# dask-contrib/dask-sql

Hardware: NVIDIA H100
Metric: rows/s on Q3-shaped filter->join->groupby (higher is better)
Workload: dtype f64

## Files before the change

### dask-sql_b200/_lib.py

```python
import ctypes as C
import os

HERE = os.path.dirname(os.path.abspath(__file__))
LIB_PATH = os.environ.get("B200SQL_LIB") or os.path.join(HERE, "libb200sql.so")

I64, F64, U8 = 0, 1, 2
U32 = 3
COL_SENTINEL = 1
MAX_COLS, MAX_TERMS, MAX_AGGS, MAX_KEYS, MAX_GATHER, MAX_PROG = 16, 8, 8, 4, 8, 64
TILE = 4096
EQ, NE, LT, LE, GT, GE, IS_NULL, IS_NOT_NULL, IS_TRUE = range(9)
AGG_SUM, AGG_SUMF, AGG_MIN, AGG_MAX, AGG_COUNT, AGG_AND, AGG_OR, AGG_XOR = range(8)
JOIN_INNER, JOIN_LEFT, JOIN_SEMI, JOIN_ANTI = range(4)
EMPTY_KEY = -(1 << 63)

OP_LOAD, OP_CONST_I, OP_CONST_F, OP_CONST_NULL, OP_I2F, OP_F2I = 0, 1, 2, 3, 4, 5
OP_ADD_I, OP_SUB_I, OP_MUL_I, OP_DIV_I, OP_NEG_I, OP_ABS_I, OP_MOD_I = 10, 11, 12, 13, 14, 15, 16
OP_ADD_F, OP_SUB_F, OP_MUL_F, OP_DIV_F, OP_NEG_F, OP_ABS_F, OP_SQRT_F = 20, 21, 22, 23, 24, 25, 26
OP_EQ_I, OP_EQ_F = 30, 40
OP_AND, OP_OR, OP_NOT, OP_ISNULL_I, OP_ISNULL_F, OP_CASE, OP_FILLNA, OP_ORD2F = 50, 51, 52, 53, 54, 55, 56, 57


class Col(C.Structure):
    _fields_ = [("data", C.c_void_p), ("valid", C.c_void_p), ("dtype", C.c_int32), ("flags", C.c_int32)]
# ... 11 lines not shown

class Agg(C.Structure):
    _fields_ = [("col", C.c_int32), ("op", C.c_int32)]


class AggState(C.Structure):
    _fields_ = [("acc", C.c_void_p * MAX_AGGS), ("cnt", C.c_void_p * MAX_AGGS), ("rows", C.c_void_p),
                ("present", C.c_void_p), ("out_slot", C.c_void_p)]


class Instr(C.Structure):
    _fields_ = [("op", C.c_int32), ("a", C.c_int32), ("imm_i", C.c_int64), ("imm_f", C.c_double)]


class Prog(C.Structure):
    _fields_ = [("code", Instr * MAX_PROG), ("n", C.c_int32), ("out_dtype", C.c_int32)]


class JoinTable(C.Structure):
    _fields_ = [("keys", Col * MAX_KEYS), ("nkeys", C.c_int32), ("dense", C.c_int32), ("head", C.c_void_p),
                ("next", C.c_void_p), ("cap", C.c_int64), ("lookup", C.c_void_p), ("kmin", C.c_int64),
                ("range", C.c_int64)]


JA_P, JA_B, JA_MUL, JA_ADD, JA_SUB, JA_RSUB, JA_ROWS = range(7)
JA_MAX_BUILD = 4


class JoinAgg(C.Structure):
    _fields_ = [("pcol", C.c_int32), ("bcol", C.c_int32), ("combine", C.c_int32), ("op", C.c_int32)]


class StarLookup(C.Structure):
    _fields_ = [("dense", C.c_int32), ("pad_", C.c_int32), ("lookup", C.c_void_p), ("kmin", C.c_int64),
                ("range", C.c_int64), ("table_keys", C.c_void_p), ("table_slots", C.c_void_p),
                ("cap", C.c_int64), ("dir", C.c_void_p)]


MAX_PEERS, PEER_MAX_ARRAYS = 16, 2 * MAX_AGGS + 1
PEER_SUM_F64, PEER_SUM_I64, PEER_MIN_I64, PEER_MAX_I64, PEER_AND_I64, PEER_OR_I64, PEER_XOR_I64 = range(7)
PEER_PRESENT_ROWS, PEER_PRESENT_INDICATOR, PEER_PRESENT_BITMAP = 1, 2, 3


class PeerMerge(C.Structure):
    _fields_ = [("world", C.c_int32), ("rank", C.c_int32), ("narrays", C.c_int32), ("presence_kind", C.c_int32),
                ("presence_array", C.c_int32), ("ops", C.c_int32 * PEER_MAX_ARRAYS),
                ("array_off", C.c_int64 * PEER_MAX_ARRAYS), ("bitmap_off", C.c_int64), ("signal_off", C.c_int64),
                ("peer_base", C.c_void_p * MAX_PEERS), ("out", C.c_void_p * PEER_MAX_ARRAYS),
                ("out_present", C.c_void_p), ("lo", C.c_int64), ("count", C.c_int64), ("local_ready", C.c_void_p),
                ("epoch", C.c_uint64)]


assert C.sizeof(Col) == 24 and C.sizeof(Term) == 32 and C.sizeof(Scan) == 656
assert C.sizeof(AggState) == 152 and C.sizeof(Instr) == 24 and C.sizeof(Prog) == 1544
assert C.sizeof(JoinTable) == 152 and C.sizeof(StarLookup) == 64 and C.sizeof(PeerMerge) == 544


def agg_identity(op):
    return {AGG_MIN: (1 << 63) - 1, AGG_MAX: -(1 << 63), AGG_AND: -1}.get(op, 0)


class B200SqlError(RuntimeError):
    pass


def _load():
    if not os.path.exists(LIB_PATH):
# ... 51 lines not shown
    "b2_join_count": [C.POINTER(Scan), C.POINTER(C.c_int32), C.POINTER(JoinTable), C.c_int32, _P, _P],
    "b2_join_write": [C.POINTER(Scan), C.POINTER(C.c_int32), C.POINTER(JoinTable), C.c_int32, _P, _P, _P,
                      _P, _P],
    "b2_join_write_gather": [C.POINTER(Scan), C.POINTER(C.c_int32), C.POINTER(JoinTable), C.c_int32, _P, _P, _P,
                             _P, C.c_int32, C.POINTER(C.c_int32), C.POINTER(_P), C.POINTER(_P), C.c_int32,
                             C.POINTER(Col), C.POINTER(_P), C.POINTER(_P), _P],
    "b2_join_key_layout": [C.POINTER(Col), C.c_int64, C.c_int64, C.c_int64, C.POINTER(Col), C.c_int32, C.c_int64,
                           _P, _P, _P, _P],
    "b2_join_write_gather_keyed": [C.POINTER(Scan), C.POINTER(C.c_int32), C.POINTER(JoinTable), C.c_int32, _P, _P,
                                   _P, _P, C.c_int32, C.POINTER(C.c_int32), C.POINTER(_P), C.POINTER(_P),
                                   C.c_int32, C.POINTER(Col), C.POINTER(C.c_int64), C.POINTER(_P), C.POINTER(_P),
                                   _P],
    "b2_join_onepass": [C.POINTER(Scan), C.POINTER(C.c_int32), C.POINTER(JoinTable), C.c_int32, C.c_int32, _P, C.c_int32,
                        C.POINTER(C.c_int32), C.POINTER(_P), C.POINTER(_P), C.c_int32, C.POINTER(Col),
                        C.POINTER(C.c_int64), C.POINTER(_P), C.POINTER(_P), _P],
    "b2_join_agg": [C.POINTER(Scan), C.c_int32, C.POINTER(JoinTable), C.c_int32, C.POINTER(Col), C.POINTER(C.c_int64),
                    C.POINTER(JoinAgg), C.c_int32, _P, _P, C.c_int32, _P, _P],
    "b2_range_partition_hist": [C.POINTER(Scan), C.c_int32, C.c_int64, C.c_int64, C.c_int32, C.c_int32, _P, _P],
    "b2_range_partition_scan": [C.c_int32, _P, _P],
    "b2_range_partition_scatter": [C.POINTER(Scan), C.c_int32, C.c_int64, C.c_int64, C.c_int32, C.c_int32, C.c_int32,
                                   C.POINTER(C.c_int32), _P, C.POINTER(_P), _P, _P],
    "b2_range_partition": [C.POINTER(Scan), C.c_int32, C.c_int64, C.c_int64, C.c_int32, C.c_int32, C.c_int32,
                           C.POINTER(C.c_int32), _P, C.POINTER(_P), _P, _P],
    "b2_iota": [_P, C.c_int64, _P],
    "b2_bitwise_combine": [_P, _P, C.c_int64, C.c_int32, _P],
    "b2_peer_merge": [C.POINTER(PeerMerge), _P],
    "b2_sort_by": [C.POINTER(Col), C.c_int64, C.c_int32, C.c_int32, _P, _P, _P],
    "b2_dense_slots": [C.POINTER(Col), C.c_int64, C.c_int64, C.c_int32, _P, _P],
    "b2_star_build_dense": [C.POINTER(Col), _P, C.c_int64, _P, C.c_int64, C.c_int64, _P, _P, _P],
    "b2_star_build_mark": [C.POINTER(Scan), C.c_int32, C.c_int64, C.c_int64, _P, _P, _P],
    "b2_star_build_rank": [_P, C.c_int64, _P],
    "b2_star_build_fill": [C.POINTER(Scan), C.c_int32, C.c_int32, C.c_int64, C.c_int64, C.c_int64, C.c_int32, _P,
                           _P, _P],
    "b2_star_build_hash": [C.POINTER(Col), _P, C.c_int64, _P, _P, _P, C.c_int64, _P, _P],
    "b2_star_agg": [C.POINTER(Scan), C.c_int32, C.POINTER(StarLookup), C.POINTER(Agg), C.c_int32,
                    C.POINTER(AggState), _P],
}

EXPORTS = sorted(list(_SIGS) + ["b2_last_error", "b2_num_tiles", "b2_stats_ws_bytes", "b2_scan_agg_ws_bytes",
                                "b2_sort_ws_bytes", "b2_join_onepass_ws_bytes", "b2_range_partition_ws_bytes",
                                "b2_f64_to_ordered", "b2_ordered_to_f64"])


call_times = {} if os.environ.get("B200SQL_CALL_TIMES") == "1" else None


def _wrap(name):
    fn = getattr(_lib, name)
    fn.restype = C.c_int32
    fn.argtypes = _SIGS[name]

    if call_times is not None:
        import time

        def call(*args):
            t0 = time.perf_counter()
            rc = fn(*args)
            rec = call_times.setdefault(name, [0, 0.0])
            rec[0] += 1
            rec[1] += time.perf_counter() - t0
            if rc != 0:
                raise B200SqlError(f"{name} failed ({rc}): {_lib.b2_last_error().decode()}")
            return rc

        call.__name__ = name
        return call
# ... 24 lines not shown
groupby_dense_ordered = _wrap("b2_groupby_dense_ordered")
groupby_dense_grouped = _wrap("b2_groupby_dense_grouped")
groupby_dense_hot = _wrap("b2_groupby_dense_hot")
hot_slots = _wrap("b2_hot_slots")
groupby_hash1 = _wrap("b2_groupby_hash1")
groupby_hashk = _wrap("b2_groupby_hashk")
join_build = _wrap("b2_join_build")
join_build_dense = _wrap("b2_join_build_dense")
join_count = _wrap("b2_join_count")
join_write = _wrap("b2_join_write")
join_write_gather = _wrap("b2_join_write_gather")
join_write_gather_keyed = _wrap("b2_join_write_gather_keyed")
join_key_layout = _wrap("b2_join_key_layout")
join_onepass = _wrap("b2_join_onepass")
join_onepass_ws_bytes = _lib.b2_join_onepass_ws_bytes
join_agg = _wrap("b2_join_agg")
range_partition = _wrap("b2_range_partition")
range_partition_hist = _wrap("b2_range_partition_hist")
range_partition_scan = _wrap("b2_range_partition_scan")
range_partition_scatter = _wrap("b2_range_partition_scatter")
range_partition_ws_bytes = _lib.b2_range_partition_ws_bytes
iota = _wrap("b2_iota")
bitwise_combine = _wrap("b2_bitwise_combine")
peer_merge = _wrap("b2_peer_merge")
sort_by = _wrap("b2_sort_by")
_lib.b2_sort_ws_bytes.restype = C.c_int64
_lib.b2_sort_ws_bytes.argtypes = [C.c_int64]
sort_ws_bytes = _lib.b2_sort_ws_bytes
dense_slots = _wrap("b2_dense_slots")
star_build_dense = _wrap("b2_star_build_dense")
star_build_mark = _wrap("b2_star_build_mark")
star_build_rank = _wrap("b2_star_build_rank")
star_build_fill = _wrap("b2_star_build_fill")
star_build_hash = _wrap("b2_star_build_hash")
star_agg = _wrap("b2_star_agg")
num_tiles = _lib.b2_num_tiles
stats_ws_bytes = _lib.b2_stats_ws_bytes
scan_agg_ws_bytes = _lib.b2_scan_agg_ws_bytes
f64_to_ordered = _lib.b2_f64_to_ordered
ordered_to_f64 = _lib.b2_ordered_to_f64


def has_symbol(name):
    try:
        getattr(_lib, name)
        return True
    except AttributeError:
        return False
```

### dask-sql_b200/csrc/groupby.cuh

```cuda
#pragma once
#include "common.cuh"
#include "pipeline.cuh"
#include "warpagg.cuh"

#define B2_GB_R 8
#define B2_GB_ROWS_PER_BLOCK (B2_BLOCK * B2_GB_R)
#define B2_MAX_PROBE 1024

template <int R, class LD>
__device__ __forceinline__ void b2_dense_slots_of(const b2_scan_t& s, const LD& ld, int key_col, int64_t kmin,
                                                  int64_t nslots, int64_t (&slot)[R]) {
  const b2_col_t& kc = s.cols[key_col];
  bool full;
  const uint32_t bits = b2_eval_terms<R>(s, ld, full);
  int64_t key[R];
  ld.template load<R>(key_col, bits, full, key);
  uint32_t kvalid = bits;
  if (kc.valid) kvalid = b2_valid_bits<R>(kc.valid, ld.row0, bits);
#pragma unroll
  for (int j = 0; j < R; ++j) {
    slot[j] = -1;
    if ((bits >> j) & 1) {
      if (!((kvalid >> j) & 1)) slot[j] = nslots - 1;
      else {
// ... 191 lines not shown
                        const __grid_constant__ b2_keys_arg keys, int64_t* __restrict__ tk,
                        uint8_t* __restrict__ tnull, int32_t* __restrict__ tstate, int64_t cap,
                        const __grid_constant__ b2_aggs_arg aggs, const __grid_constant__ b2_aggstate_t st,
                        int32_t* __restrict__ flags) {
  auto body = [&](const auto& ld) { b2_hashk_body(s, ld, keys, tk, tnull, tstate, cap, aggs, st, flags); };
  if (PIPE) b2_tile_pipeline(s, pp, body);
  else b2_tile_direct<B2_GB_R>(s, body);
}

__global__ void __launch_bounds__(B2_BLOCK)
b2_dense_slots_kernel(const __grid_constant__ b2_col_t key, int64_t n, int64_t kmin, int32_t null_slot,
                      int32_t* __restrict__ out) {
  for (int64_t i = (int64_t)blockIdx.x * B2_BLOCK + threadIdx.x; i < n; i += (int64_t)gridDim.x * B2_BLOCK) {
    const int64_t raw = b2_load_raw(key, i);
    out[i] = b2_is_null(key, i, raw) ? null_slot : (int32_t)(raw - kmin);
  }
}

__global__ void __launch_bounds__(B2_BLOCK)
b2_star_build_dense_kernel(const __grid_constant__ b2_col_t pk, const int32_t* __restrict__ sel, int64_t n_sel,
                           const int32_t* __restrict__ slot_of_row, int64_t kmin, int64_t range,
                           int32_t* __restrict__ lookup, int32_t* __restrict__ flags) {
  for (int64_t i = (int64_t)blockIdx.x * B2_BLOCK + threadIdx.x; i < n_sel; i += (int64_t)gridDim.x * B2_BLOCK) {
    const int64_t r = sel ? sel[i] : i;
    const int64_t raw = b2_load_raw(pk, r);
    if (b2_is_null(pk, r, raw)) continue;
    const uint64_t d = (uint64_t)raw - (uint64_t)kmin;
    if (d >= (uint64_t)range) continue;
    const int32_t old = atomicExch(lookup + d, slot_of_row[i]);
    if (old != -1) flags[0] = 1;
  }
}

template <bool FILL>
__global__ void __launch_bounds__(B2_BLOCK)
b2_star_build_scan_kernel(const __grid_constant__ b2_scan_t s, int pk_col, int grp_col, int64_t pk_min,
                          int64_t pk_range, int64_t grp_min, int32_t null_slot, uint64_t* __restrict__ dir,
                          int32_t* __restrict__ slots, int32_t* __restrict__ flags) {
  const int tile_off = (threadIdx.x >> 5) * (32 * B2_GB_R) + (threadIdx.x & 31);
  const b2_col_t& pc = s.cols[pk_col];
  const b2_col_t& gc = s.cols[grp_col];
  for (int64_t base = (int64_t)blockIdx.x * B2_GB_ROWS_PER_BLOCK; base < s.n;
       base += (int64_t)gridDim.x * B2_GB_ROWS_PER_BLOCK) {
    const b2_gld ld{&s, base + tile_off};
    bool full;
    const uint32_t bits = b2_eval_terms<B2_GB_R>(s, ld, full);
    int64_t pk[B2_GB_R];
    ld.template load<B2_GB_R>(pk_col, bits, full, pk);
    uint32_t live = bits;
    if (pc.valid) live &= b2_valid_bits<B2_GB_R>(pc.valid, ld.row0, bits);
#pragma unroll
    for (int j = 0; j < B2_GB_R; ++j) {
      const uint64_t d = (uint64_t)pk[j] - (uint64_t)pk_min;
      if (!(((live >> j) & 1) && d < (uint64_t)pk_range)) live &= ~(1u << j);
    }
    if (!FILL) {
#pragma unroll
      for (int j = 0; j < B2_GB_R; ++j) {
        if (!((live >> j) & 1)) continue;
        const uint64_t d = (uint64_t)pk[j] - (uint64_t)pk_min;
        const uint32_t b = 1u << (d & 31);
        if (atomicOr(reinterpret_cast<uint32_t*>(dir + (d >> 5)), b) & b) flags[0] = 1;
      }
    } else {
      int64_t grp[B2_GB_R];
      ld.template load<B2_GB_R>(grp_col, live, false, grp);
      uint32_t gnull = 0;
      if (gc.valid) gnull = live & ~b2_valid_bits<B2_GB_R>(gc.valid, ld.row0, live);
#pragma unroll
      for (int j = 0; j < B2_GB_R; ++j) {
        if (!((live >> j) & 1)) continue;
        const uint64_t d = (uint64_t)pk[j] - (uint64_t)pk_min;
        const uint64_t w = dir[d >> 5];
        const uint32_t pos = (uint32_t)(w >> 32) + __popc((uint32_t)w & ((1u << (d & 31)) - 1));
        slots[pos] = (gnull >> j) & 1 ? null_slot : (int32_t)(grp[j] - grp_min);
      }
    }
  }
}

struct b2_scan_io_dir {
  uint64_t* dir;
  __device__ int64_t get(int64_t i) const { return __popc((uint32_t)dir[i]); }
  __device__ void put(int64_t i, int64_t v) const { dir[i] = (uint64_t)(uint32_t)dir[i] | ((uint64_t)v << 32); }
};

__global__ void __launch_bounds__(B2_SCAN_THREADS) b2_star_build_rank_kernel(uint64_t* __restrict__ dir, int64_t nwords) {
  b2_block_exclusive_scan(b2_scan_io_dir{dir}, nwords);
}

__global__ void __launch_bounds__(B2_BLOCK)
b2_star_build_hash_kernel(const __grid_constant__ b2_col_t pk, const int32_t* __restrict__ sel, int64_t n_sel,
                          const int32_t* __restrict__ slot_of_row, int64_t* __restrict__ tk,
                          int32_t* __restrict__ ts, int64_t cap, int32_t* __restrict__ flags) {
  for (int64_t i = (int64_t)blockIdx.x * B2_BLOCK + threadIdx.x; i < n_sel; i += (int64_t)gridDim.x * B2_BLOCK) {
    const int64_t r = sel ? sel[i] : i;
    const int64_t key = b2_load_raw(pk, r);
    if (b2_is_null(pk, r, key)) continue;
    if (key == B2_EMPTY_KEY) { flags[1] = 1; continue; }
    uint64_t h = b2_mix64((uint64_t)key) & (uint64_t)(cap - 1);
    bool done = false;
    for (int probe = 0; probe < B2_MAX_PROBE && !done; ++probe) {
      const unsigned long long old = atomicCAS(reinterpret_cast<unsigned long long*>(tk + h),
                                               (unsigned long long)B2_EMPTY_KEY, (unsigned long long)key);
      if (old == (unsigned long long)B2_EMPTY_KEY) { ts[h] = slot_of_row[i]; done = true; }
      else if (old == (unsigned long long)key) { flags[0] = 1; done = true; }
      else h = (h + 1) & (uint64_t)(cap - 1);
    }
// ... 2 lines not shown
}

__device__ __forceinline__ int32_t b2_star_lookup(const b2_starlookup_t& lk, int64_t key) {
  if (lk.dense) {
    const uint64_t d = (uint64_t)key - (uint64_t)lk.kmin;
    return d < (uint64_t)lk.range ? b2_ld_keep_i32(lk.lookup + d) : -1;
  }
  uint64_t h = b2_mix64((uint64_t)key) & (uint64_t)(lk.cap - 1);
  for (int probe = 0; probe < B2_MAX_PROBE; ++probe) {
    const int64_t cur = __ldg(reinterpret_cast<const long long*>(lk.table_keys) + h);
    if (cur == key) return b2_ld_keep_i32(lk.table_slots + h);
    if (cur == B2_EMPTY_KEY) return -1;
    h = (h + 1) & (uint64_t)(lk.cap - 1);
  }
  return -1;
}

#define B2_STAR_R 16
template <int R, class LD>
__device__ __forceinline__ void b2_star_body(const b2_scan_t& s, const LD& ld, int fk_col, const b2_starlookup_t& lk,
                                             const b2_aggs_arg& aggs, const b2_aggstate_t& st) {
  const b2_col_t& kc = s.cols[fk_col];
  bool full0;
  const uint32_t inb = b2_bounds_bits<R>(ld.row0, s.n, full0);
  int64_t key[R];
  ld.template load<R>(fk_col, inb, full0, key);
  bool full;
  const uint32_t bits = b2_eval_terms<R>(s, ld, full);
  uint32_t live = bits;
  if (kc.valid) live &= b2_valid_bits<R>(kc.valid, ld.row0, bits);
  const bool prefetch = aggs.n > 0 && aggs.a[0].col >= 0;
  int64_t pre[R];
  int32_t found[R];
  if (lk.dense == 2) {
    const uint64_t range = (uint64_t)lk.range;
    uint64_t w[R];
#pragma unroll
    for (int j = 0; j < R; ++j) {
      const uint64_t d = (uint64_t)key[j] - (uint64_t)lk.kmin;
      w[j] = (((live >> j) & 1) && d < range) ? (uint64_t)b2_ld_keep_i64(reinterpret_cast<const int64_t*>(lk.dir) + (d >> 5)) : 0;
    }
    if (prefetch) ld.template load<R>(aggs.a[0].col, live, false, pre);
#pragma unroll
    for (int j = 0; j < R; ++j) {
      const uint32_t b = (uint32_t)((uint64_t)key[j] - (uint64_t)lk.kmin) & 31;
      const uint32_t bits = (uint32_t)w[j];
      found[j] = (bits >> b) & 1 ? b2_ld_keep_i32(lk.lookup + (uint32_t)(w[j] >> 32) + __popc(bits & ((1u << b) - 1))) : -1;
    }
  } else if (lk.dense) {
    const uint64_t range = (uint64_t)lk.range;
#pragma unroll
    for (int j = 0; j < R; ++j) {
      const uint64_t d = (uint64_t)key[j] - (uint64_t)lk.kmin;
      found[j] = (((live >> j) & 1) && d < range) ? b2_ld_keep_i32(lk.lookup + d) : -1;
    }
  } else {
#pragma unroll
    for (int j = 0; j < R; ++j) {
      found[j] = -1;
      if (((live >> j) & 1) && key[j] != B2_EMPTY_KEY) found[j] = b2_star_lookup(lk, key[j]);
    }
  }
  if (lk.dense != 2 && prefetch) ld.template load<R>(aggs.a[0].col, live, false, pre);
  int64_t slot[R];
#pragma unroll
  for (int j = 0; j < R; ++j) slot[j] = found[j];
  b2_apply_aggs<R>(s, ld, aggs.a, aggs.n, st, slot, pre);
}

template <bool PIPE>
__global__ void __launch_bounds__(PIPE ? B2_PIPE_THREADS : B2_BLOCK)
b2_star_agg_kernel(const __grid_constant__ b2_scan_t s, const __grid_constant__ b2_pipe_t pp, int fk_col,
                   const __grid_constant__ b2_starlookup_t lk, const __grid_constant__ b2_aggs_arg aggs,
                   const __grid_constant__ b2_aggstate_t st) {
  if (PIPE) b2_tile_pipeline(s, pp, [&](const auto& ld) { b2_star_body<B2_PIPE_R>(s, ld, fk_col, lk, aggs, st); });
  else b2_tile_direct<B2_STAR_R>(s, [&](const auto& ld) { b2_star_body<B2_STAR_R>(s, ld, fk_col, lk, aggs, st); });
}

extern "C" {

static int32_t b2_check_state(const b2_aggs_arg& aa, const b2_aggstate_t* st) {
  B2_REQUIRE(st, "null aggstate");
  for (int a = 0; a < aa.n; ++a) {
    if (aa.a[a].col < 0) { B2_REQUIRE(st->rows, "COUNT(*) needs aggstate.rows"); continue; }
    if (aa.a[a].op == B2_AGG_COUNT) B2_REQUIRE(st->cnt[a], "COUNT needs a cnt array");
    else B2_REQUIRE(st->acc[a], "aggregate needs an acc array");
  }
  return B2_OK;
}
static inline bool b2_pow2(int64_t x) { return x > 0 && (x & (x - 1)) == 0; }

static int32_t b2_groupby_dense_impl(const b2_scan_t* scan, int32_t key_col, int64_t kmin, int64_t nslots,
                                     const b2_agg_t* aggs, int32_t naggs, const b2_aggstate_t* st,
                                     unsigned long long* ticket, void* stream) {
  int32_t rc = b2_check_scan(scan);
  if (rc) return rc;
  b2_aggs_arg aa;
// ... 156 lines not shown
    int64_t nblk = (scan->n + B2_GB_ROWS_PER_BLOCK - 1) / B2_GB_ROWS_PER_BLOCK;
    int grid = b2_wave_grid(b2_groupby_hashk_kernel<false>, B2_BLOCK, nblk);
    b2_groupby_hashk_kernel<false><<<grid, B2_BLOCK, 0, (cudaStream_t)stream>>>(*scan, pp, ka, table_keys, table_nulls,
                                                                        table_state, cap, aa, *st, d_flags);
  }
  B2_CHECK_LAUNCH("b2_groupby_hashk_kernel");
  return B2_OK;
}

int32_t b2_dense_slots(const b2_col_t* key, int64_t n, int64_t kmin, int32_t null_slot, int32_t* out_slot,
                       void* stream) {
  B2_REQUIRE(key && out_slot, "null argument");
  if (n <= 0) return B2_OK;
  int grid = b2_wave_grid(b2_dense_slots_kernel, B2_BLOCK, (n + B2_BLOCK - 1) / B2_BLOCK);
  b2_dense_slots_kernel<<<grid, B2_BLOCK, 0, (cudaStream_t)stream>>>(*key, n, kmin, null_slot, out_slot);
  B2_CHECK_LAUNCH("b2_dense_slots_kernel");
  return B2_OK;
}

int32_t b2_star_build_dense(const b2_col_t* pk, const int32_t* sel, int64_t n_sel, const int32_t* slot_of_row,
                            int64_t kmin, int64_t range, int32_t* lookup, int32_t* d_flags, void* stream) {
  B2_REQUIRE(pk && slot_of_row && lookup && d_flags, "null argument");
  B2_REQUIRE(pk->dtype == B2_I64, "dense lookup needs an int64 key");
  if (n_sel <= 0) return B2_OK;
  int grid = b2_wave_grid(b2_star_build_dense_kernel, B2_BLOCK, (n_sel + B2_BLOCK - 1) / B2_BLOCK);
  b2_star_build_dense_kernel<<<grid, B2_BLOCK, 0, (cudaStream_t)stream>>>(*pk, sel, n_sel, slot_of_row, kmin,
                                                                           range, lookup, d_flags);
  B2_CHECK_LAUNCH("b2_star_build_dense_kernel");
  return B2_OK;
}

static int32_t b2_star_build_pass(bool fill, const b2_scan_t* scan, int32_t pk_col, int32_t grp_col,
                                  int64_t pk_min, int64_t pk_range, int64_t grp_min, int32_t null_slot,
                                  uint64_t* dir, int32_t* slots, int32_t* d_flags, void* stream) {
  int32_t rc = b2_check_scan(scan);
  if (rc) return rc;
  B2_REQUIRE(pk_col >= 0 && pk_col < scan->ncols && grp_col >= 0 && grp_col < scan->ncols, "column out of range");
  B2_REQUIRE(scan->cols[pk_col].dtype == B2_I64 && scan->cols[grp_col].dtype == B2_I64, "dense keys must be int64");
  B2_REQUIRE(pk_range > 0 && pk_range < ((int64_t)1 << 31), "bad range");
  if (scan->n == 0) return B2_OK;
  int64_t nblk = (scan->n + B2_GB_ROWS_PER_BLOCK - 1) / B2_GB_ROWS_PER_BLOCK;
  if (fill) {
    int grid = b2_wave_grid(b2_star_build_scan_kernel<true>, B2_BLOCK, nblk);
    b2_star_build_scan_kernel<true><<<grid, B2_BLOCK, 0, (cudaStream_t)stream>>>(*scan, pk_col, grp_col, pk_min, pk_range,
                                                                                  grp_min, null_slot, dir, slots, d_flags);
  } else {
    int grid = b2_wave_grid(b2_star_build_scan_kernel<false>, B2_BLOCK, nblk);
    b2_star_build_scan_kernel<false><<<grid, B2_BLOCK, 0, (cudaStream_t)stream>>>(*scan, pk_col, grp_col, pk_min, pk_range,
                                                                                   grp_min, null_slot, dir, slots, d_flags);
  }
  B2_CHECK_LAUNCH("b2_star_build_scan_kernel");
  return B2_OK;
}

int32_t b2_star_build_mark(const b2_scan_t* scan, int32_t pk_col, int64_t pk_min, int64_t pk_range, uint64_t* dir,
                           int32_t* d_flags, void* stream) {
  B2_REQUIRE(dir && d_flags, "null argument");
  return b2_star_build_pass(false, scan, pk_col, pk_col, pk_min, pk_range, 0, 0, dir, nullptr, d_flags, stream);
}

int32_t b2_star_build_rank(uint64_t* dir, int64_t pk_range, void* stream) {
  B2_REQUIRE(dir, "null argument");
  B2_REQUIRE(pk_range > 0 && pk_range < ((int64_t)1 << 31), "bad range");
  b2_star_build_rank_kernel<<<1, B2_SCAN_THREADS, 0, (cudaStream_t)stream>>>(dir, (pk_range + 31) / 32);
  B2_CHECK_LAUNCH("b2_star_build_rank_kernel");
  return B2_OK;
}

int32_t b2_star_build_fill(const b2_scan_t* scan, int32_t pk_col, int32_t grp_col, int64_t pk_min,
                           int64_t pk_range, int64_t grp_min, int32_t null_slot, const uint64_t* dir,
                           int32_t* slots, void* stream) {
  B2_REQUIRE(dir && slots, "null argument");
  return b2_star_build_pass(true, scan, pk_col, grp_col, pk_min, pk_range, grp_min, null_slot,
                            const_cast<uint64_t*>(dir), slots, nullptr, stream);
}

int32_t b2_star_build_hash(const b2_col_t* pk, const int32_t* sel, int64_t n_sel, const int32_t* slot_of_row,
                           int64_t* table_keys, int32_t* table_slots, int64_t cap, int32_t* d_flags,
                           void* stream) {
  B2_REQUIRE(pk && slot_of_row && table_keys && table_slots && d_flags, "null argument");
  B2_REQUIRE(pk->dtype == B2_I64, "star lookup needs an int64 key");
  B2_REQUIRE(b2_pow2(cap), "cap must be a power of two");
  if (n_sel <= 0) return B2_OK;
  int grid = b2_wave_grid(b2_star_build_hash_kernel, B2_BLOCK, (n_sel + B2_BLOCK - 1) / B2_BLOCK);
  b2_star_build_hash_kernel<<<grid, B2_BLOCK, 0, (cudaStream_t)stream>>>(*pk, sel, n_sel, slot_of_row, table_keys,
                                                                          table_slots, cap, d_flags);
  B2_CHECK_LAUNCH("b2_star_build_hash_kernel");
  return B2_OK;
}

int32_t b2_star_agg(const b2_scan_t* scan, int32_t fk_col, const b2_starlookup_t* lk, const b2_agg_t* aggs,
                    int32_t naggs, const b2_aggstate_t* st, void* stream) {
  int32_t rc = b2_check_scan(scan);
  if (rc) return rc;
  b2_aggs_arg aa;
  if ((rc = b2_check_aggs(scan, aggs, naggs, &aa))) return rc;
  if ((rc = b2_check_state(aa, st))) return rc;
  B2_REQUIRE(lk, "null lookup");
  B2_REQUIRE(fk_col >= 0 && fk_col < scan->ncols, "fk column out of range");
  B2_REQUIRE(scan->cols[fk_col].dtype == B2_I64, "fk must be int64");
  B2_REQUIRE(lk->dense >= 0 && lk->dense <= 2, "bad lookup kind");
  if (lk->dense == 2) B2_REQUIRE(lk->dir && lk->lookup && lk->range > 0 && lk->range < ((int64_t)1 << 31), "bad bitmap lookup");
  else if (lk->dense) B2_REQUIRE(lk->lookup && lk->range > 0, "bad dense lookup");
  else B2_REQUIRE(lk->table_keys && lk->table_slots && b2_pow2(lk->cap), "bad hash lookup");
  if (scan->n == 0) return B2_OK;
  b2_pipe_t pp;
  b2_make_pipe(*scan, &pp);
  if (pp.enabled) {
    int grid = b2_pipe_grid(b2_star_agg_kernel<true>, pp, scan->n);
    b2_star_agg_kernel<true><<<grid, B2_PIPE_THREADS, pp.smem_bytes, (cudaStream_t)stream>>>(*scan, pp, fk_col, *lk, aa, *st);
  } else {
    int64_t nblk = (scan->n + (int64_t)B2_BLOCK * B2_STAR_R - 1) / ((int64_t)B2_BLOCK * B2_STAR_R);
    int grid = b2_wave_grid(b2_star_agg_kernel<false>, B2_BLOCK, nblk);
    b2_star_agg_kernel<false><<<grid, B2_BLOCK, 0, (cudaStream_t)stream>>>(*scan, pp, fk_col, *lk, aa, *st);
  }
  B2_CHECK_LAUNCH("b2_star_agg_kernel");
  return B2_OK;
}

}
```

### dask-sql_b200/executor.py

```python
import ctypes as C
import os
from typing import Dict, List, Optional, Sequence, Set

import numpy as np
import torch

from . import _lib as L
from . import device as D
from . import expr as E
from . import parallel as P
from .device import DeviceColumn, TermSpec, I64, F64, U8
from .expr import Expr, ColRef, Lit, Call
from .frame import LazyFrame, Source, TableSource, JoinSource, AggSource, SortSource, LimitSource
from .table import DeviceTable, HostColumn

DENSE_MAX_SLOTS = 1 << 27
_TORCH_DT = {I64: torch.int64, F64: torch.float64, U8: torch.uint8}
_LOGICAL = {I64: "int64", F64: "float64", U8: "bool"}

stats = {"launches": 0, "star_fused": 0, "dense_groupby": 0, "hash_groupby": 0, "dense_join": 0,
         "chain_join": 0, "keyed_join": 0, "partitioned_groupby": 0, "h2d_bytes": 0, "d2h_bytes": 0}


kernel_events = None
# ... 1468 lines not shown
        self.gname = src.group_cols[0]
        self.gexpr0 = gexpr0
        self.glog = dim.col_type(gexpr0.name)[1] if isinstance(gexpr0, ColRef) else "int64"
        self.plan = AggPlan([(E.substitute(e, fact.exprs) if e is not None else None, o, f) for e, o, f in aggs],
                            _nullable_fn(fact, sharded))
        if any(not isinstance(ka.expr, ColRef) for ka in self.plan.kaggs):
            raise _NotPreparable()
        self.keep = []
        self.dim_launch = []
        if owner:
            needed = {pk_e.name, ge.name}
            for p in dpred:
                p.refs(needed)
            for part in self._resident_parts(dim.source.table, needed):
                ctx = ScanCtx(part, dpred)
                pk_slot, g_slot = ctx.slot(pk_e), ctx.slot(ge)
                self._only_table_columns(ctx)
                self.dim_launch.append((ctx.scan(), pk_slot, g_slot))
                self.keep.append(ctx)
        needed = set(fk_e.refs())
        for ka in self.plan.kaggs:
            ka.expr.refs(needed)
        for p in fpred:
            p.refs(needed)
        self.fact_launch = []
        for part in self._resident_parts(fact.source.table, needed):
            ctx = ScanCtx(part, fpred)
            fk_slot = ctx.slot(fk_e)
            specs = [(ctx.slot(ka.expr), ka.op) for ka in self.plan.kaggs]
            self._only_table_columns(ctx)
            self.fact_launch.append((ctx.scan(), fk_slot, D.make_aggs(specs), len(specs), part.n))
            self.keep.append(ctx)
        self.dn = dn
        _, self.flags_off, words = _star_bitmap_words(self.prange, dn)
        self.lookup = torch.empty(words, dtype=torch.int32, device=dev)
        self.lk = _star_bitmap_lookup(self.lookup, self.pmin, self.prange, dn)
        self.tabs = [GroupState(dev, self.nslots, self.plan, need_present=True,
                                alloc=_padded_slots(self.nslots, sharded))]
        self.refill = [self._refill_list(self.tabs[0].table)]
        self.dirty = [False]
        self.peer = None
        self.epoch = 0
        self.free = [None, None]
        self.merge_bufs = {}
        self.runs = 0

    @staticmethod
    def _refill_list(t: D.GroupTable):
        out = []
        for acc in t.acc:
            if acc is not None:
                out.append((acc, float(acc[0].item()) if acc.dtype == torch.float64 else int(acc[0].item())))
        for cnt in t.cnt:
            if cnt is not None:
                out.append((cnt, 0))
        if t.rows is not None:
            out.append((t.rows, 0))
        if t.present is not None:
            out.append((t.present, 0))
        return out

    def install_peer_merge(self, state):
        self.tabs, self.refill, self.dirty, self.peer, self.arena, self.local_ready = state
        stats["peer_merge_plans"] = stats.get("peer_merge_plans", 0) + 1

    def build_peer_merge(self):
        rank, size = P.world()
        dev = self.dev
        alloc = _padded_slots(self.nslots, True)
# ... 59 lines not shown

    @staticmethod
    def _resident_parts(table, needed):
        parts = []
        for p in table.partitions:
            n = next(iter(p.values())).n if p else 0
            if n == 0:
                continue
            cols = {}
            for name in needed:
                c = p[name]
                if not isinstance(c, DeviceColumn):
                    raise _NotPreparable()
                cols[name] = c
            parts.append(Part(cols, n))
        return parts

    @staticmethod
    def _only_table_columns(ctx: "ScanCtx"):
        if any(not k.startswith("col:") for k in ctx.index):
            raise _NotPreparable()

    def run(self, src) -> Part:
        i = self.runs & 1
        self.runs += 1
        buf = self.lookup
        main = D.cur_stream()
        sp = D.stream_ptr()
        if self.free[i] is not None:
            self.free[i].synchronize()
        if self.owner:
            with _Phase("build"):
                _star_bitmap_build(buf, self.dim_launch, self.pmin, self.prange, self.gmin, self.nslots - 1,
                                   self.dn, sp)
        if self.bcast:
            with _Phase("bcast"):
                P.broadcast_(buf, 0)
        ti = i if self.peer is not None else 0
        t = self.tabs[ti].table
        with _Phase("scan"):
            if self.dirty[ti]:
                for tensor, value in self.refill[ti]:
                    tensor.fill_(value)
            self.dirty[ti] = True
            for scan, fk_slot, aggs_arr, naggs, n in self.fact_launch:
                stats["launches"] += 1
                ev = _kernel_event_begin("b2_star_agg_kernel", n)
                L.star_agg(C.byref(scan), fk_slot, C.byref(self.lk), aggs_arr, naggs, C.byref(t.state), sp)
                _kernel_event_end(ev)
        if self.peer is not None:
            m, view = self.peer[ti]
            self.epoch += 1
            m.epoch = self.epoch
            with _Phase("peer_merge"):
                stats["launches"] += 1
                ev = _kernel_event_begin("b2_peer_merge_kernel", m.count)
                L.peer_merge(C.byref(m), sp)
                _kernel_event_end(ev)
        else:
            view = _merge_dense(t, self.plan, self.sharded, self.dev, keep=self.merge_bufs)
        stats["star_fused"] += 1

        def general():
            stats["star_fused"] -= 1
            return run_aggregate(src, allow_fast=False)

        out = _finalize_dense(view, self.gmin, self.gname, self.gexpr0, self.glog, self.plan, self.dev,
                              key_nullable=self.gnull, check=buf[self.flags_off:], fallback=general)
        done = torch.cuda.Event()
        done.record(main)
        self.free[i] = done
        return out


class _NotPreparable(Exception):
    pass


def _star_bitmap_words(prange, dn):
    slots = 2 * ((prange + 31) // 32)
    flags = slots + min(dn, prange)
    return slots, flags, flags + 4


def _star_bitmap_lookup(buf, pmin, prange, dn):
    lk = L.StarLookup()
    lk.dense, lk.dir, lk.kmin, lk.range = 2, buf.data_ptr(), pmin, prange
    lk.lookup = buf.data_ptr() + 4 * _star_bitmap_words(prange, dn)[0]
    return lk


def _star_bitmap_build(buf, launches, pmin, prange, gmin, null_slot, dn, sp):
    slots_off, flags_off, _ = _star_bitmap_words(prange, dn)
    base = buf.data_ptr()
    dirp, slots, flags = C.c_void_p(base), C.c_void_p(base + 4 * slots_off), C.c_void_p(base + 4 * flags_off)
    L.memset(dirp, 0, 4 * slots_off, sp)
    L.memset(flags, 0, 16, sp)
    for scan, pk_slot, _ in launches:
        stats["launches"] += 1
        L.star_build_mark(C.byref(scan), pk_slot, pmin, prange, dirp, flags, sp)
    stats["launches"] += 1
    L.star_build_rank(dirp, prange, sp)
    for scan, pk_slot, g_slot in launches:
        stats["launches"] += 1
        L.star_build_fill(C.byref(scan), pk_slot, g_slot, pmin, prange, gmin, null_slot, dirp, slots, sp)


def _star_dense_fast(src, fact, dim, fk_e, pk_e, gexprs, aggs, fact_pred, dim_pred, sharded, dev) -> Optional[Part]:
    if len(gexprs) != 1 or not isinstance(dim.source, TableSource) or not isinstance(pk_e, ColRef):
        return None
    ge = E.substitute(gexprs[0], dim.exprs)
    if not isinstance(ge, ColRef) or ge.dtype != I64 or pk_e.dtype != I64:
        return None
    rank, world = P.world()
    dist = frame_distribution(dim)
    if world > 1 and dist == "sharded":
        return None
    table = dim.source.table
    owner = world == 1 or dist != "root" or rank == 0
    meta = None
    if owner:
        pst, gst = table.column_stats(pk_e.name), table.column_stats(ge.name)
        gnull = table.column_nullable(ge.name)
        meta = (pst.vmin, pst.vmax, gst.vmin, gst.vmax, table.nrows, gnull)
    if world > 1 and dist == "root":
        cache = table.__dict__.setdefault("_root_meta", {})
        ck = (pk_e.name, ge.name)
        if ck not in cache:
            cache[ck] = P.broadcast_object(meta, 0)
        meta = cache[ck]
    pmin, pmax, gmin, gmax, dn, gnull = meta
    if pmin is None or gmin is None or dn == 0:
        return None
    prange, grng = pmax - pmin + 1, gmax - gmin + 1
    if not (prange <= max(4 * dn, 1 << 16) and prange < (1 << 31)):
        return None
    if not (grng + 1 <= DENSE_MAX_SLOTS and grng <= 8 * dn + 1024):
        return None
    dpred, never = simplify_pred(dim.pred + [E.substitute(p, dim.exprs) for p in dim_pred])
    fpred, fnever = simplify_pred(fact.pred + [E.substitute(p, fact.exprs) for p in fact_pred])
    if never or fnever:
        return None
    nslots = grng + 1
    if os.environ.get("B200SQL_NO_PREPARED") != "1":
        prep = PreparedStar.get(src, fact, dim, fk_e, pk_e, ge, gexprs[0], aggs, fpred, dpred,
                                (pmin, prange, gmin, grng, gnull, dn), owner, world > 1 and dist == "root", sharded, dev)
        if prep is not None:
            return prep.run(src)
    _, flags_off, words = _star_bitmap_words(prange, dn)
    buf = torch.empty(words, dtype=torch.int32, device=dev)
    flags = buf[flags_off:]
    with _Phase("build"):
        if owner:
            needed: Set[str] = {pk_e.name, ge.name}
            for p in dpred:
                p.refs(needed)
            launches, keep = [], []
            for part in materialize(dim.source, needed):
                if part.n == 0:
                    continue
                ctx = ScanCtx(part, dpred)
                pk_slot, g_slot = ctx.slot(pk_e), ctx.slot(ge)
                launches.append((ctx.scan(), pk_slot, g_slot))
                keep.append(ctx)
            _star_bitmap_build(buf, launches, pmin, prange, gmin, nslots - 1, dn, D.stream_ptr())
    if world > 1 and dist == "root":
        with _Phase("bcast"):
            P.broadcast_(buf, 0)
    plan = AggPlan([(E.substitute(e, fact.exprs) if e is not None else None, o, f) for e, o, f in aggs],
                   _nullable_fn(fact, sharded))
    gs = GroupState(dev, nslots, plan, need_present=True, alloc=_padded_slots(nslots, sharded))
    lk = _star_bitmap_lookup(buf, pmin, prange, dn)
    needed = set(fk_e.refs())
    for ka in plan.kaggs:
        ka.expr.refs(needed)
    for p in fpred:
        p.refs(needed)
    with _Phase("scan"):
        for part in materialize(fact.source, needed, pred=fpred):
            if part.n == 0:
                continue
            ctx = ScanCtx(part, fpred)
            fk_slot = ctx.slot(fk_e)
            gs.bind(ctx)
            stats["launches"] += 1
            ev = _kernel_event_begin("b2_star_agg_kernel", part.n)
            L.star_agg(C.byref(ctx.scan()), fk_slot, C.byref(lk), gs.table.aggs, len(gs.table.specs),
                       C.byref(gs.table.state), D.stream_ptr())
            _kernel_event_end(ev)
    view = _merge_dense(gs.table, plan, sharded, dev)
    glog = dim.col_type(gexprs[0].name)[1] if isinstance(gexprs[0], ColRef) else "int64"
    stats["star_fused"] += 1

    def general():
        stats["star_fused"] -= 1
        return run_aggregate(src, allow_fast=False)

    return _finalize_dense(view, gmin, src.group_cols[0], gexprs[0], glog, plan, dev, key_nullable=gnull,
                           check=flags, fallback=general)


def try_star(src: AggSource, child: LazyFrame, gexprs, aggs, pred, sharded, allow_fast=True) -> Optional[Part]:
    js: JoinSource = child.source
    if js.how != "inner" or len(js.left_on) != 1 or any(fn.lower() in MOMENT_FUNCS for _, _, fn in aggs):
        return None
# ... 467 lines not shown
```

### include/b200sql.h

```cpp
#ifndef B200SQL_H
#define B200SQL_H
#include <stdint.h>
#ifdef __cplusplus
extern "C" {
#endif

#define B2_OK            0
#define B2_ERR_CUDA     -1
#define B2_ERR_ARG      -2

#define B2_I64 0
#define B2_F64 1
#define B2_U8  2
#define B2_U32 3

#define B2_MAX_COLS   16
#define B2_MAX_TERMS   8
#define B2_MAX_AGGS    8
#define B2_MAX_KEYS    4
#define B2_MAX_GATHER  8
#define B2_MAX_PROG   64
#define B2_TILE     4096

#define B2_EQ 0
// ... 256 lines not shown
                    int64_t* d_out_acc, int64_t* d_out_cnt, int32_t accumulate, void* ws, void* stream);

int32_t b2_groupby_dense_ordered(const b2_scan_t* scan, int32_t key_col, int64_t kmin, int64_t nslots,
                                 const b2_agg_t* aggs, int32_t naggs, const b2_aggstate_t* st, uint64_t* d_ticket,
                                 void* stream);
int64_t b2_range_partition_ws_bytes(int32_t nbuckets);
int32_t b2_range_partition_hist(const b2_scan_t* scan, int32_t key_col, int64_t kmin, int64_t nslots, int32_t shift,
                                int32_t nbuckets, void* d_ws, void* stream);
int32_t b2_range_partition_scan(int32_t nbuckets, void* d_ws, void* stream);
int32_t b2_range_partition_scatter(const b2_scan_t* scan, int32_t key_col, int64_t kmin, int64_t nslots, int32_t shift,
                                   int32_t nbuckets, int32_t ncarry, const int32_t* carry_cols, int64_t* out_key,
                                   void* const* out_cols, void* d_ws, void* stream);
int32_t b2_range_partition(const b2_scan_t* scan, int32_t key_col, int64_t kmin, int64_t nslots, int32_t shift,
                           int32_t nbuckets, int32_t ncarry, const int32_t* carry_cols, int64_t* out_key,
                           void* const* out_cols, void* d_ws, void* stream);

int64_t b2_sort_ws_bytes(int64_t n);
int32_t b2_iota(int32_t* out, int64_t n, void* stream);
int32_t b2_sort_by(const b2_col_t* col, int64_t n, int32_t descending, int32_t nulls_first, int32_t* idx,
                   void* ws, void* stream);

int32_t b2_dense_slots(const b2_col_t* key, int64_t n, int64_t kmin, int32_t null_slot,
                       int32_t* out_slot, void* stream);

int32_t b2_star_build_dense(const b2_col_t* pk, const int32_t* sel, int64_t n_sel,
                            const int32_t* slot_of_row, int64_t kmin, int64_t range,
                            int32_t* lookup, int32_t* d_flags, void* stream);
int32_t b2_star_build_mark(const b2_scan_t* scan, int32_t pk_col, int64_t pk_min, int64_t pk_range,
                           uint64_t* dir, int32_t* d_flags, void* stream);
int32_t b2_star_build_rank(uint64_t* dir, int64_t pk_range, void* stream);
int32_t b2_star_build_fill(const b2_scan_t* scan, int32_t pk_col, int32_t grp_col, int64_t pk_min,
                           int64_t pk_range, int64_t grp_min, int32_t null_slot, const uint64_t* dir,
                           int32_t* slots, void* stream);
int32_t b2_star_build_hash(const b2_col_t* pk, const int32_t* sel, int64_t n_sel,
                           const int32_t* slot_of_row, int64_t* table_keys, int32_t* table_slots,
                           int64_t cap, int32_t* d_flags, void* stream);

typedef struct b2_starlookup {
  int32_t dense;
  int32_t pad_;
  const int32_t* lookup;
  int64_t kmin;
  int64_t range;
  const int64_t* table_keys;
  const int32_t* table_slots;
  int64_t cap;
  const uint64_t* dir;
} b2_starlookup_t;

int32_t b2_star_agg(const b2_scan_t* scan, int32_t fk_col, const b2_starlookup_t* lk,
                    const b2_agg_t* aggs, int32_t naggs, const b2_aggstate_t* st, void* stream);

#ifdef __cplusplus
}
#endif
#endif
```

Before: 75.14 billion.

## Bit-pack star-join slot lookup into 16 or 21-bit fields

Stores the dimension-to-group slot array of the bitmap star lookup in packed 64-bit words, with 16 or 21 bits per entry when the group count fits, instead of int32 per entry. The build fill kernel writes entries with atomicCAS read-modify-write, and the fact-side probe extracts the field with a shift and mask. The aim is a smaller lookup that stays resident in L2 and cuts probe traffic, at the cost of extra build atomics, a divide-by-3 trick for 21-bit packing, and 64-bit probe loads.

```diff
diff --git a/dask-sql_b200/_lib.py b/dask-sql_b200/_lib.py
--- a/dask-sql_b200/_lib.py
+++ b/dask-sql_b200/_lib.py
@@ -67,7 +67,7 @@
 
 
 class StarLookup(C.Structure):
-    _fields_ = [("dense", C.c_int32), ("pad_", C.c_int32), ("lookup", C.c_void_p), ("kmin", C.c_int64),
+    _fields_ = [("dense", C.c_int32), ("slot_bits", C.c_int32), ("lookup", C.c_void_p), ("kmin", C.c_int64),
                 ("range", C.c_int64), ("table_keys", C.c_void_p), ("table_slots", C.c_void_p),
                 ("cap", C.c_int64), ("dir", C.c_void_p)]
 
@@ -185,6 +185,8 @@
     "b2_star_build_rank": [_P, C.c_int64, _P],
     "b2_star_build_fill": [C.POINTER(Scan), C.c_int32, C.c_int32, C.c_int64, C.c_int64, C.c_int64, C.c_int32, _P,
                            _P, _P],
+    "b2_star_build_fill_packed": [C.POINTER(Scan), C.c_int32, C.c_int32, C.c_int64, C.c_int64, C.c_int64,
+                                  C.c_int32, _P, _P, C.c_int32, _P],
     "b2_star_build_hash": [C.POINTER(Col), _P, C.c_int64, _P, _P, _P, C.c_int64, _P, _P],
     "b2_star_agg": [C.POINTER(Scan), C.c_int32, C.POINTER(StarLookup), C.POINTER(Agg), C.c_int32,
                     C.POINTER(AggState), _P],
@@ -275,6 +277,7 @@
 star_build_mark = _wrap("b2_star_build_mark")
 star_build_rank = _wrap("b2_star_build_rank")
 star_build_fill = _wrap("b2_star_build_fill")
+star_build_fill_packed = _wrap("b2_star_build_fill_packed")
 star_build_hash = _wrap("b2_star_build_hash")
 star_agg = _wrap("b2_star_agg")
 num_tiles = _lib.b2_num_tiles
diff --git a/dask-sql_b200/csrc/groupby.cuh b/dask-sql_b200/csrc/groupby.cuh
--- a/dask-sql_b200/csrc/groupby.cuh
+++ b/dask-sql_b200/csrc/groupby.cuh
@@ -247,11 +247,15 @@
   }
 }
 
+__device__ __forceinline__ uint32_t b2_slot_word(uint32_t pos, int slot_bits) {
+  return slot_bits == 16 ? pos >> 2 : __umulhi(pos, 0x55555556u);
+}
+
 template <bool FILL>
 __global__ void __launch_bounds__(B2_BLOCK)
 b2_star_build_scan_kernel(const __grid_constant__ b2_scan_t s, int pk_col, int grp_col, int64_t pk_min,
                           int64_t pk_range, int64_t grp_min, int32_t null_slot, uint64_t* __restrict__ dir,
-                          int32_t* __restrict__ slots, int32_t* __restrict__ flags) {
+                          void* __restrict__ slots, int slot_bits, int32_t* __restrict__ flags) {
   const int tile_off = (threadIdx.x >> 5) * (32 * B2_GB_R) + (threadIdx.x & 31);
   const b2_col_t& pc = s.cols[pk_col];
   const b2_col_t& gc = s.cols[grp_col];
@@ -288,7 +292,18 @@
         const uint64_t d = (uint64_t)pk[j] - (uint64_t)pk_min;
         const uint64_t w = dir[d >> 5];
         const uint32_t pos = (uint32_t)(w >> 32) + __popc((uint32_t)w & ((1u << (d & 31)) - 1));
-        slots[pos] = (gnull >> j) & 1 ? null_slot : (int32_t)(grp[j] - grp_min);
+        const int32_t v = (gnull >> j) & 1 ? null_slot : (int32_t)(grp[j] - grp_min);
+        if (slot_bits == 32) {
+          static_cast<int32_t*>(slots)[pos] = v;
+        } else {
+          const uint32_t q = b2_slot_word(pos, slot_bits);
+          const uint32_t sh = (pos - q * (64 / slot_bits)) * slot_bits;
+          unsigned long long* p = reinterpret_cast<unsigned long long*>(slots) + q;
+          const unsigned long long m = ((1ull << slot_bits) - 1) << sh;
+          const unsigned long long e = ((unsigned long long)(uint32_t)v << sh) & m;
+          unsigned long long old = 0, seen;
+          while ((seen = atomicCAS(p, old, (old & ~m) | e)) != old) old = seen;
+        }
       }
     }
   }
@@ -357,6 +372,7 @@
   const bool prefetch = aggs.n > 0 && aggs.a[0].col >= 0;
   int64_t pre[R];
   int32_t found[R];
+  int64_t slot[R];
   if (lk.dense == 2) {
     const uint64_t range = (uint64_t)lk.range;
     uint64_t w[R];
@@ -366,11 +382,34 @@
       w[j] = (((live >> j) & 1) && d < range) ? (uint64_t)b2_ld_keep_i64(reinterpret_cast<const int64_t*>(lk.dir) + (d >> 5)) : 0;
     }
     if (prefetch) ld.template load<R>(aggs.a[0].col, live, false, pre);
-#pragma unroll
-    for (int j = 0; j < R; ++j) {
-      const uint32_t b = (uint32_t)((uint64_t)key[j] - (uint64_t)lk.kmin) & 31;
-      const uint32_t bits = (uint32_t)w[j];
-      found[j] = (bits >> b) & 1 ? b2_ld_keep_i32(lk.lookup + (uint32_t)(w[j] >> 32) + __popc(bits & ((1u << b) - 1))) : -1;
+    const int sb = lk.slot_bits;
+    if (sb == 32) {
+#pragma unroll
+      for (int j = 0; j < R; ++j) {
+        const uint32_t b = (uint32_t)((uint64_t)key[j] - (uint64_t)lk.kmin) & 31;
+        const uint32_t bits = (uint32_t)w[j];
+        found[j] = (bits >> b) & 1 ? b2_ld_keep_i32(lk.lookup + (uint32_t)(w[j] >> 32) + __popc(bits & ((1u << b) - 1))) : -1;
+      }
+    } else {
+      const int k = 64 / sb;
+      const uint64_t* words = reinterpret_cast<const uint64_t*>(lk.lookup);
+#pragma unroll
+      for (int j = 0; j < R; ++j) {
+        const uint32_t b = (uint32_t)((uint64_t)key[j] - (uint64_t)lk.kmin) & 31;
+        const uint32_t bits = (uint32_t)w[j];
+        found[j] = -1;
+        slot[j] = 0;
+        if ((bits >> b) & 1) {
+          const uint32_t pos = (uint32_t)(w[j] >> 32) + __popc(bits & ((1u << b) - 1));
+          const uint32_t q = b2_slot_word(pos, sb);
+          found[j] = (int32_t)((pos - q * k) * sb);
+          slot[j] = b2_ld_keep_i64(reinterpret_cast<const int64_t*>(words + q));
+        }
+      }
+      const uint64_t mask = (1ull << sb) - 1;
+#pragma unroll
+      for (int j = 0; j < R; ++j)
+        found[j] = found[j] < 0 ? -1 : (int32_t)(((uint64_t)slot[j] >> found[j]) & mask);
     }
   } else if (lk.dense) {
     const uint64_t range = (uint64_t)lk.range;
@@ -387,7 +426,6 @@
     }
   }
   if (lk.dense != 2 && prefetch) ld.template load<R>(aggs.a[0].col, live, false, pre);
-  int64_t slot[R];
 #pragma unroll
   for (int j = 0; j < R; ++j) slot[j] = found[j];
   b2_apply_aggs<R>(s, ld, aggs.a, aggs.n, st, slot, pre);
@@ -610,7 +648,7 @@
 
 static int32_t b2_star_build_pass(bool fill, const b2_scan_t* scan, int32_t pk_col, int32_t grp_col,
                                   int64_t pk_min, int64_t pk_range, int64_t grp_min, int32_t null_slot,
-                                  uint64_t* dir, int32_t* slots, int32_t* d_flags, void* stream) {
+                                  uint64_t* dir, void* slots, int32_t slot_bits, int32_t* d_flags, void* stream) {
   int32_t rc = b2_check_scan(scan);
   if (rc) return rc;
   B2_REQUIRE(pk_col >= 0 && pk_col < scan->ncols && grp_col >= 0 && grp_col < scan->ncols, "column out of range");
@@ -621,11 +659,11 @@
   if (fill) {
     int grid = b2_wave_grid(b2_star_build_scan_kernel<true>, B2_BLOCK, nblk);
     b2_star_build_scan_kernel<true><<<grid, B2_BLOCK, 0, (cudaStream_t)stream>>>(*scan, pk_col, grp_col, pk_min, pk_range,
-                                                                                  grp_min, null_slot, dir, slots, d_flags);
+                                                                                  grp_min, null_slot, dir, slots, slot_bits, d_flags);
   } else {
     int grid = b2_wave_grid(b2_star_build_scan_kernel<false>, B2_BLOCK, nblk);
     b2_star_build_scan_kernel<false><<<grid, B2_BLOCK, 0, (cudaStream_t)stream>>>(*scan, pk_col, grp_col, pk_min, pk_range,
-                                                                                   grp_min, null_slot, dir, slots, d_flags);
+                                                                                   grp_min, null_slot, dir, slots, slot_bits, d_flags);
   }
   B2_CHECK_LAUNCH("b2_star_build_scan_kernel");
   return B2_OK;
@@ -634,7 +672,7 @@
 int32_t b2_star_build_mark(const b2_scan_t* scan, int32_t pk_col, int64_t pk_min, int64_t pk_range, uint64_t* dir,
                            int32_t* d_flags, void* stream) {
   B2_REQUIRE(dir && d_flags, "null argument");
-  return b2_star_build_pass(false, scan, pk_col, pk_col, pk_min, pk_range, 0, 0, dir, nullptr, d_flags, stream);
+  return b2_star_build_pass(false, scan, pk_col, pk_col, pk_min, pk_range, 0, 0, dir, nullptr, 32, d_flags, stream);
 }
 
 int32_t b2_star_build_rank(uint64_t* dir, int64_t pk_range, void* stream) {
@@ -648,9 +686,19 @@
 int32_t b2_star_build_fill(const b2_scan_t* scan, int32_t pk_col, int32_t grp_col, int64_t pk_min,
                            int64_t pk_range, int64_t grp_min, int32_t null_slot, const uint64_t* dir,
                            int32_t* slots, void* stream) {
+  return b2_star_build_fill_packed(scan, pk_col, grp_col, pk_min, pk_range, grp_min, null_slot, dir,
+                                   reinterpret_cast<uint64_t*>(slots), 32, stream);
+}
+
+int32_t b2_star_build_fill_packed(const b2_scan_t* scan, int32_t pk_col, int32_t grp_col, int64_t pk_min,
+                                  int64_t pk_range, int64_t grp_min, int32_t null_slot, const uint64_t* dir,
+                                  uint64_t* slots, int32_t slot_bits, void* stream) {
   B2_REQUIRE(dir && slots, "null argument");
+  B2_REQUIRE(slot_bits == 16 || slot_bits == 21 || slot_bits == 32, "slot_bits must be 16, 21 or 32");
+  B2_REQUIRE(slot_bits == 32 || (null_slot >= 0 && null_slot < (1 << slot_bits)), "null_slot does not fit slot_bits");
+  B2_REQUIRE(slot_bits == 32 || ((uintptr_t)slots & 7) == 0, "packed slots must be 8-byte aligned");
   return b2_star_build_pass(true, scan, pk_col, grp_col, pk_min, pk_range, grp_min, null_slot,
-                            const_cast<uint64_t*>(dir), slots, nullptr, stream);
+                            const_cast<uint64_t*>(dir), slots, slot_bits, nullptr, stream);
 }
 
 int32_t b2_star_build_hash(const b2_col_t* pk, const int32_t* sel, int64_t n_sel, const int32_t* slot_of_row,
@@ -678,19 +726,25 @@
   B2_REQUIRE(fk_col >= 0 && fk_col < scan->ncols, "fk column out of range");
   B2_REQUIRE(scan->cols[fk_col].dtype == B2_I64, "fk must be int64");
   B2_REQUIRE(lk->dense >= 0 && lk->dense <= 2, "bad lookup kind");
-  if (lk->dense == 2) B2_REQUIRE(lk->dir && lk->lookup && lk->range > 0 && lk->range < ((int64_t)1 << 31), "bad bitmap lookup");
-  else if (lk->dense) B2_REQUIRE(lk->lookup && lk->range > 0, "bad dense lookup");
-  else B2_REQUIRE(lk->table_keys && lk->table_slots && b2_pow2(lk->cap), "bad hash lookup");
+  b2_starlookup_t l = *lk;
+  if (l.dense == 2) {
+    B2_REQUIRE(l.dir && l.lookup && l.range > 0 && l.range < ((int64_t)1 << 31), "bad bitmap lookup");
+    if (l.slot_bits == 0) l.slot_bits = 32;
+    B2_REQUIRE(l.slot_bits == 16 || l.slot_bits == 21 || l.slot_bits == 32, "slot_bits must be 0, 16, 21 or 32");
+    B2_REQUIRE(l.slot_bits == 32 || ((uintptr_t)l.lookup & 7) == 0, "packed slots must be 8-byte aligned");
+  }
+  else if (l.dense) B2_REQUIRE(l.lookup && l.range > 0, "bad dense lookup");
+  else B2_REQUIRE(l.table_keys && l.table_slots && b2_pow2(l.cap), "bad hash lookup");
   if (scan->n == 0) return B2_OK;
   b2_pipe_t pp;
   b2_make_pipe(*scan, &pp);
   if (pp.enabled) {
     int grid = b2_pipe_grid(b2_star_agg_kernel<true>, pp, scan->n);
-    b2_star_agg_kernel<true><<<grid, B2_PIPE_THREADS, pp.smem_bytes, (cudaStream_t)stream>>>(*scan, pp, fk_col, *lk, aa, *st);
+    b2_star_agg_kernel<true><<<grid, B2_PIPE_THREADS, pp.smem_bytes, (cudaStream_t)stream>>>(*scan, pp, fk_col, l, aa, *st);
   } else {
     int64_t nblk = (scan->n + (int64_t)B2_BLOCK * B2_STAR_R - 1) / ((int64_t)B2_BLOCK * B2_STAR_R);
     int grid = b2_wave_grid(b2_star_agg_kernel<false>, B2_BLOCK, nblk);
-    b2_star_agg_kernel<false><<<grid, B2_BLOCK, 0, (cudaStream_t)stream>>>(*scan, pp, fk_col, *lk, aa, *st);
+    b2_star_agg_kernel<false><<<grid, B2_BLOCK, 0, (cudaStream_t)stream>>>(*scan, pp, fk_col, l, aa, *st);
   }
   B2_CHECK_LAUNCH("b2_star_agg_kernel");
   return B2_OK;
diff --git a/dask-sql_b200/executor.py b/dask-sql_b200/executor.py
--- a/dask-sql_b200/executor.py
+++ b/dask-sql_b200/executor.py
@@ -1524,9 +1524,10 @@
             self.fact_launch.append((ctx.scan(), fk_slot, D.make_aggs(specs), len(specs), part.n))
             self.keep.append(ctx)
         self.dn = dn
-        _, self.flags_off, words = _star_bitmap_words(self.prange, dn)
+        self.slot_bits = _star_slot_bits(self.nslots - 1)
+        _, self.flags_off, words = _star_bitmap_words(self.prange, dn, self.slot_bits)
         self.lookup = torch.empty(words, dtype=torch.int32, device=dev)
-        self.lk = _star_bitmap_lookup(self.lookup, self.pmin, self.prange, dn)
+        self.lk = _star_bitmap_lookup(self.lookup, self.pmin, self.prange, dn, self.slot_bits)
         self.tabs = [GroupState(dev, self.nslots, self.plan, need_present=True,
                                 alloc=_padded_slots(self.nslots, sharded))]
         self.refill = [self._refill_list(self.tabs[0].table)]
@@ -1652,7 +1653,7 @@
         if self.owner:
             with _Phase("build"):
                 _star_bitmap_build(buf, self.dim_launch, self.pmin, self.prange, self.gmin, self.nslots - 1,
-                                   self.dn, sp)
+                                   self.dn, self.slot_bits, sp)
         if self.bcast:
             with _Phase("bcast"):
                 P.broadcast_(buf, 0)
@@ -1697,24 +1698,29 @@
     pass
 
 
-def _star_bitmap_words(prange, dn):
+def _star_slot_bits(null_slot):
+    return 16 if null_slot < (1 << 16) else 21 if null_slot < (1 << 21) else 32
+
+
+def _star_bitmap_words(prange, dn, slot_bits):
     slots = 2 * ((prange + 31) // 32)
-    flags = slots + min(dn, prange)
+    k = 64 // slot_bits
+    flags = slots + 2 * ((min(dn, prange) + k - 1) // k)
     return slots, flags, flags + 4
 
 
-def _star_bitmap_lookup(buf, pmin, prange, dn):
+def _star_bitmap_lookup(buf, pmin, prange, dn, slot_bits):
     lk = L.StarLookup()
-    lk.dense, lk.dir, lk.kmin, lk.range = 2, buf.data_ptr(), pmin, prange
-    lk.lookup = buf.data_ptr() + 4 * _star_bitmap_words(prange, dn)[0]
+    lk.dense, lk.dir, lk.kmin, lk.range, lk.slot_bits = 2, buf.data_ptr(), pmin, prange, slot_bits
+    lk.lookup = buf.data_ptr() + 4 * _star_bitmap_words(prange, dn, slot_bits)[0]
     return lk
 
 
-def _star_bitmap_build(buf, launches, pmin, prange, gmin, null_slot, dn, sp):
-    slots_off, flags_off, _ = _star_bitmap_words(prange, dn)
+def _star_bitmap_build(buf, launches, pmin, prange, gmin, null_slot, dn, slot_bits, sp):
+    slots_off, flags_off, _ = _star_bitmap_words(prange, dn, slot_bits)
     base = buf.data_ptr()
     dirp, slots, flags = C.c_void_p(base), C.c_void_p(base + 4 * slots_off), C.c_void_p(base + 4 * flags_off)
-    L.memset(dirp, 0, 4 * slots_off, sp)
+    L.memset(dirp, 0, 4 * (flags_off if slot_bits < 32 else slots_off), sp)
     L.memset(flags, 0, 16, sp)
     for scan, pk_slot, _ in launches:
         stats["launches"] += 1
@@ -1723,7 +1729,8 @@
     L.star_build_rank(dirp, prange, sp)
     for scan, pk_slot, g_slot in launches:
         stats["launches"] += 1
-        L.star_build_fill(C.byref(scan), pk_slot, g_slot, pmin, prange, gmin, null_slot, dirp, slots, sp)
+        L.star_build_fill_packed(C.byref(scan), pk_slot, g_slot, pmin, prange, gmin, null_slot, dirp, slots,
+                                 slot_bits, sp)
 
 
 def _star_dense_fast(src, fact, dim, fk_e, pk_e, gexprs, aggs, fact_pred, dim_pred, sharded, dev) -> Optional[Part]:
@@ -1767,7 +1774,8 @@
                                 (pmin, prange, gmin, grng, gnull, dn), owner, world > 1 and dist == "root", sharded, dev)
         if prep is not None:
             return prep.run(src)
-    _, flags_off, words = _star_bitmap_words(prange, dn)
+    slot_bits = _star_slot_bits(nslots - 1)
+    _, flags_off, words = _star_bitmap_words(prange, dn, slot_bits)
     buf = torch.empty(words, dtype=torch.int32, device=dev)
     flags = buf[flags_off:]
     with _Phase("build"):
@@ -1783,14 +1791,14 @@
                 pk_slot, g_slot = ctx.slot(pk_e), ctx.slot(ge)
                 launches.append((ctx.scan(), pk_slot, g_slot))
                 keep.append(ctx)
-            _star_bitmap_build(buf, launches, pmin, prange, gmin, nslots - 1, dn, D.stream_ptr())
+            _star_bitmap_build(buf, launches, pmin, prange, gmin, nslots - 1, dn, slot_bits, D.stream_ptr())
     if world > 1 and dist == "root":
         with _Phase("bcast"):
             P.broadcast_(buf, 0)
     plan = AggPlan([(E.substitute(e, fact.exprs) if e is not None else None, o, f) for e, o, f in aggs],
                    _nullable_fn(fact, sharded))
     gs = GroupState(dev, nslots, plan, need_present=True, alloc=_padded_slots(nslots, sharded))
-    lk = _star_bitmap_lookup(buf, pmin, prange, dn)
+    lk = _star_bitmap_lookup(buf, pmin, prange, dn, slot_bits)
     needed = set(fk_e.refs())
     for ka in plan.kaggs:
         ka.expr.refs(needed)
diff --git a/include/b200sql.h b/include/b200sql.h
--- a/include/b200sql.h
+++ b/include/b200sql.h
@@ -312,13 +312,16 @@
 int32_t b2_star_build_fill(const b2_scan_t* scan, int32_t pk_col, int32_t grp_col, int64_t pk_min,
                            int64_t pk_range, int64_t grp_min, int32_t null_slot, const uint64_t* dir,
                            int32_t* slots, void* stream);
+int32_t b2_star_build_fill_packed(const b2_scan_t* scan, int32_t pk_col, int32_t grp_col, int64_t pk_min,
+                                  int64_t pk_range, int64_t grp_min, int32_t null_slot, const uint64_t* dir,
+                                  uint64_t* slots, int32_t slot_bits, void* stream);
 int32_t b2_star_build_hash(const b2_col_t* pk, const int32_t* sel, int64_t n_sel,
                            const int32_t* slot_of_row, int64_t* table_keys, int32_t* table_slots,
                            int64_t cap, int32_t* d_flags, void* stream);
 
 typedef struct b2_starlookup {
   int32_t dense;
-  int32_t pad_;
+  int32_t slot_bits;
   const int32_t* lookup;
   int64_t kmin;
   int64_t range;
```

After: 77.77 billion, median of 6. 3.5% higher.
